# roncapat/UNIGE-TASI-path-planners

Measured on AMD Instinct MI355X. Metric: grid cells updated/sec (full plan + 100 replans), 4096^2 map, higher is better.
Workload: dtype f32

## Files before the change

unige-tasi-path-planners_amd/csrc/ufm_host.h:

```cpp
#pragma once

#define HIPCHK(expr)                                                      \
    do {                                                                  \
        hipError_t _e = (expr);                                           \
        if (_e != hipSuccess) return UFM_ERR_HIP_BASE - (int)_e;          \
    } while (0)

#include "ufm_route.h"
#include "ufm_path.h"

static_assert(RJOBS <= ROUTE_MAX_JOBS && RTMAX >= 3, "ufm_route.h places at most ROUTE_MAX_JOBS blocks");
constexpr RouteConfig ROUTE_CONFIG{T, RTMAX, RJOBS, ROUTE_MAX_RECTS, 65 * 65};

template <int V> using IntC = std::integral_constant<int, V>;
template <class F> void with_lower_op(int algo, F &&f) {
    if (algo == UFM_ALGO_FD) f(IntC<UFM_ALGO_FD>{});
    else if (algo == UFM_ALGO_SG) f(IntC<UFM_ALGO_SG>{});
    else f(IntC<ALGO_DFM1>{});
}
template <class F> void with_raise_op(int algo, bool follow_info, F &&f) {
    if (algo == UFM_ALGO_DFM && follow_info) f(IntC<ALGO_DFM1_INFO>{});
    else with_lower_op(algo, f);
}
template <class F> void with_elements(int algo, F &&f) {
// ... 962 lines not shown
            const int cnt = (p.h + 1) * (p.w + 1);
            if (pl.fused) put_rect(r.rb.rect[r.rb.nrect++], p);
            else k_clear_marks<<<(cnt + 255) / 256, 256, 0, stream>>>(P, p.m, p.x, p.y, p.w, p.h);
        }
        pending.resize(kept);
    }
    return UFM_OK;
}

int Engine::fused_end(float band) {
    ++pub_seq;
    k_replan_end<<<64, T * T, 0, stream>>>(P, iter[Q_RAISE], iter[Q_LOWER], band, h_ctr, h_flag, pub_seq);
    finalize_bp(1);
    HIPCHK(hipGetLastError());
    return wait_published();
}

int Engine::submit_block(StepRun &r) {
    const StepPlan &pl = r.plan;
    const bool batch = pl.route == Route::BlockBatch;
    RegionJobs rjs{};
    rjs.n = pl.njobs;
    const unsigned int seq = ++pub_seq;
    for (int i = 0; i < pl.njobs; ++i) {
        const RouteJob &pj = pl.job[i];
        RegionJob &j = rjs.j[i];
        if (batch) {
            j.rb.sb = step_begin_of(pj.map, 1, 0);
            j.rb.nrect = pj.nrect;
            std::memcpy(j.rb.rect, pj.rect, sizeof(pj.rect));
        } else {
            j.rb = r.rb;
        }
        j.rb.k_raise = iter[Q_RAISE]; j.rb.band = r.band;
        j.tx0 = pj.tx0; j.ntx = pj.ntx; j.ty0 = pj.ty0; j.nty = pj.nty;
        j.dyn = r.dyn_now; j.k_lower = iter[Q_LOWER]; j.max_sweeps = region_sweeps; j.debug = region_debug;
        j.slack = 255.0f * SQRT2F + 1.0f;
        j.delta = region_band > 0.0f ? region_band * 4.0f * mean_cost : INFINITY;
        j.map = pj.map; j.batch = batch ? 1 : 0; j.seq = seq;
    }
    if (pl.held_in_kernel) {
        const int first = r.rb.nrect - (int)lazy.size();
        for (size_t i = 0; i < lazy.size(); ++i) rjs.j[0].psrc[first + (int)i] = h_lazy + (size_t)lazy[i].slot * 4096;
        lazy.clear();
    }
    if (batch) {
        HIPCHK(hipMemsetAsync(&P.ctr->rbound, 0, offsetof(DevCounters, done_fail) + sizeof(int) - offsetof(DevCounters, rbound), stream));
        k_fill<<<1, 64, 0, stream>>>(reinterpret_cast<float *>(&P.ctr->qmin[Q_RAISE]), (size_t)1, INFINITY);
    }
    if (batch) flush_dyn(r);
    else { dyn_dev = r.dyn_now; r.dyn_pending = false; }
    const bool reg_timed = profiling && (region_runs & 7u) == 0u;
    if (reg_timed) for (auto &e : reg_ev) if (!e) HIPCHK(hipEventCreate(&e));
    with_raise_op(algo, dfm_follow_info, [&](auto a) {
        launch(k_replan_region<a()>, dim3(rjs.n), dim3(NTHR), stream, reg_timed ? reg_ev[0] : nullptr, reg_timed ? reg_ev[1] : nullptr, P, rjs, h_ctr, h_flag);
    });
    HIPCHK(hipGetLastError());
    last_active = 1;
    { int rc = wait_published(); if (rc != UFM_OK) return rc; }
    ufm_stats &st = r.st;
    st.region_launches = 1u;
    for (int i = 0; i < rjs.n; ++i) st.region_tiles += (uint32_t)(rjs.j[i].ntx * rjs.j[i].nty);
    if (reg_timed) {
        hipError_t q;
        while ((q = hipEventQuery(reg_ev[1])) == hipErrorNotReady) __builtin_ia32_pause();
        HIPCHK(q);
        HIPCHK(hipEventElapsedTime(&st.region_kernel_ms, reg_ev[0], reg_ev[1]));
        st.region_timed = 1u;
    }
    region_runs += (uint32_t)rjs.n;
    if (h_ctr->done) region_done += (uint32_t)rjs.n;
    else if (focused) {
        float qm;
        std::memcpy(&qm, &h_ctr->qmin[Q_RAISE], sizeof(float));
        r.skip_raise = !(qm < h_ctr->rbound);
    }
    return UFM_OK;
}

int Engine::continue_block(StepRun &r) {
    const int nr2 = r.skip_raise ? 1 : std::max(1, cont_raise), nl2 = cont_lower;
    last_active = 1;
    k_unpark<<<1, 1024, 0, stream>>>(P, Q_RAISE, iter[Q_RAISE], -1.0f);
    for (int i = 0; i < nr2; ++i) launch_relax(MODE_RAISE, -1.0f);
    k_raise_to_lower<<<1, 1024, 0, stream>>>(P, iter[Q_LOWER]);
    for (int i = 0; i < nl2; ++i) launch_relax(MODE_LOWER, INFINITY);
    { int rc = fused_end(r.band); if (rc != UFM_OK) return rc; }
    r.fast_done = h_ctr->done != 0;
    r.st.raise_launches += (uint32_t)nr2;
    r.st.launches += (uint32_t)(nr2 + nl2);
    r.skip_raise = false;
    ++region_cont; if (r.fast_done) ++region_cont_done;
    return UFM_OK;
}

int Engine::submit_graph(StepRun &r) {
    r.rb.k_raise = iter[Q_RAISE]; r.rb.band = r.band;
    hipGraphExec_t ge = nullptr;
    { int rc = replan_graph(r.nr, r.nl, r.band, &ge); if (rc != UFM_OK) return rc; }
    h_job->rb = r.rb; h_job->k_lower = iter[Q_LOWER]; h_job->seq = ++pub_seq;
    h_job->dyn = r.dyn_now; dyn_dev = r.dyn_now; r.dyn_pending = false;
    __atomic_thread_fence(__ATOMIC_RELEASE);
    HIPCHK(hipGraphLaunch(ge, stream));
    iter[Q_RAISE] += r.nr; iter[Q_LOWER] += r.nl;
    last_active = 1;
    return wait_published();
}

// ... 757 lines not shown
```

unige-tasi-path-planners_amd/csrc/ufm_region.h:

```cpp

constexpr int UFM_REGION_PRIO = 2;
#define UFM_REGION_SETPRIO(x) __builtin_amdgcn_s_setprio(x)
constexpr int UFM_REGION_IDLE_SLEEP = 8;
constexpr int UFM_REGION_IDLE_SLEEP_RAISE = 8;
constexpr int RTMAX = 128 / T;
constexpr int RN = RTMAX * T;
constexpr int RP = RN + 8;
constexpr int RCP = RN + 4;
constexpr int RBP = RN;
constexpr int TP = T / 4;
constexpr int RPW = RTMAX * TP / 4;
constexpr int RWW = (RPW * RPW + 31) / 32;
constexpr int RFRAME = 4 * RTMAX + 4;

struct RegionJob {
    ReplanBegin rb;
    DevDyn dyn;
    int tx0, ty0, ntx, nty;
    int k_lower;
    unsigned int seq;
    int max_sweeps;
    int debug;
    float slack;
    float delta;
    int map;
    int batch;
    const uint8_t *psrc[4];
};
constexpr int RJOBS = 8;
struct RegionJobs { int n; RegionJob j[RJOBS]; };

__device__ __forceinline__ int prio_read_fresh(const DevParams &P, int qz, int kk, int gt) {
    const unsigned long long v = __hip_atomic_load(&P.prio[(size_t)(qz * 2 + (kk & 1)) * P.NT + gt], __ATOMIC_RELAXED, __HIP_MEMORY_SCOPE_AGENT);
    return (int)(v >> 32) == 0x7FFFFFFF - kk ? (int)(unsigned int)v : INFBITS;
}

struct RegionShared {
    int wake[16][RWW];
    int ever[16][RWW];
    int renew[16][RWW];
    int tbp[RTMAX * RTMAX];
    int seed[16][RWW];
    int defer[2][16][RWW];
    int dprio[2][RTMAX * RTMAX];
    int tflag[RTMAX * RTMAX];
    int traised[RTMAX * RTMAX];
    int actL[RFRAME], actR[RFRAME];
    int soff[4];
    float sdist[4];
    float B0, rbound;
    float theta;
    float Bgate;
    int rmin;
    float Bsub;
    int swas[4];
    int idle, giveup, again, any_start_in;
    unsigned long long sweeps;
    int expanded;
    int m_r, m_l, done;
    int dkey;
    int dbg[8];
    int dbg2[8];
    unsigned long long tstamp[12];
};

__device__ __forceinline__ float region_start_key(const float *Gs, const RegionShared &S) {
    if (!S.any_start_in) return S.B0;
    float b = 0.0f;
#pragma unroll
    for (int i = 0; i < 4; ++i) {
        const int o = S.soff[i];
        if (o < 0) continue;
        const float g = Gs[o];
        if (g < INFINITY) b = fmaxf(b, g + S.sdist[i]);
    }
    return b > 0.0f ? b : INFINITY;
}

__device__ __forceinline__ float region_lower_bound(const float *Gs, const RegionShared &S) {
    if (!S.any_start_in) return S.B0;
    float b = 0.0f;
    bool pending = false;
#pragma unroll
    for (int i = 0; i < 4; ++i) {
        const int o = S.soff[i];
        if (o < 0) continue;
        const float g = Gs[o];
        if (g < INFINITY) b = fmaxf(b, g + S.sdist[i]);
        else if (S.swas[i]) pending = true;
    }
    if (pending) return fmaxf(b, S.rbound);
    return b > 0.0f ? b : INFINITY;
}

template <int ALGOF, int MODE>
__device__ void region_phase(const DevParams &P, const RegionJob &J, float *Gs, const uint8_t *Cb, uint8_t *Bb, RegionShared &S,
                             int thr, float hm, int focused, int goal_lx, int goal_ly) {
    constexpr int ALGO = algo_of(ALGOF);
    constexpr bool FOLLOW = (ALGOF & ALGO_FOLLOW_INFO) != 0;
    constexpr bool BPRAISE = MODE == MODE_RAISE && (!is_dfm<ALGO> || FOLLOW);
    const int tid = threadIdx.x, w = wave_index16(tid >> 6), lane = tid & 63;
    const int q = lane & 3, nd = lane >> 2;
    const int nprow = J.ntx * TP, npcol = J.nty * TP;
    unsigned long long wake_sel = 0ull;
    if (lane < 9) {
        const int dr = lane / 3 - 1, dc = lane % 3 - 1;
        wake_sel = ~0ull;
        if (dr < 0) wake_sel &= 0x000000000000FFFFull; else if (dr > 0) wake_sel &= 0xFFFF000000000000ull;
        if (dc < 0) wake_sel &= 0x000F000F000F000Full; else if (dc > 0) wake_sel &= 0xF000F000F000F000ull;
    }
    const int colour = ((nd >> 2) & 1) | ((nd & 1) << 1);
    const bool wt_lane = lane < 9;
    const int wt_dr = wt_lane ? lane / 3 - 1 : 0, wt_dc = wt_lane ? lane % 3 - 1 : 0;
    const int wt_ar = (w >> 2) + wt_dr, wt_ac = (w & 3) + wt_dc;
    const int wt_wave = ((wt_ar & 3) << 2) | (wt_ac & 3), wt_di = (wt_ar >> 2) * RPW + (wt_ac >> 2);
    const float sx = J.rb.sb.sx, sy = J.rb.sb.sy;
    const int rx0 = J.tx0 * T, ry0 = J.ty0 * T;
    int budget = J.max_sweeps;
    unsigned int my_sweeps = 0;
    auto cost_at = [=](int r, int c) { const int b = Cb[r * RCP + c]; return b >= thr ? INFINITY : (float)b; };
    const int so0 = __builtin_amdgcn_readfirstlane(S.soff[0]), so1 = __builtin_amdgcn_readfirstlane(S.soff[1]);
    const int so2 = __builtin_amdgcn_readfirstlane(S.soff[2]), so3 = __builtin_amdgcn_readfirstlane(S.soff[3]);
    const bool dbg_nogate = (J.debug & 1) != 0, dbg_count = (J.debug & 2) != 0;
    const float Bphase = (MODE == MODE_LOWER) ? S.Bgate : INFINITY;
    const float rb_phase = S.rbound + J.slack;
    const int nwords = min(RWW, (((nprow + 3) / 4 - 1) * RPW + (npcol + 3) / 4 + 31) / 32);
    UFM_REGION_SETPRIO(UFM_REGION_PRIO);
    for (;;) {
        bool took = false;
        bool vote = __hip_atomic_load(&S.giveup, __ATOMIC_RELAXED, __HIP_MEMORY_SCOPE_WORKGROUP) != 0;
        for (int wd = 0; wd < nwords && !vote; ++wd) {
            if (__hip_atomic_load(&S.wake[w][wd], __ATOMIC_RELAXED, __HIP_MEMORY_SCOPE_WORKGROUP) == 0) continue;
            int bits = 0;
            if (lane == 0) bits = atomicExch(&S.wake[w][wd], 0);
            bits = __builtin_amdgcn_readfirstlane(bits);
            if (!bits) continue;
            if (MODE == MODE_RAISE && lane == 0) S.ever[w][wd] |= bits;
            int seedbits = 0;
            if (BPRAISE) seedbits = __builtin_amdgcn_readfirstlane(S.seed[w][wd]) & bits;
            while (bits) {
                const int j = __ffs(bits) - 1;
                if (budget <= 0) {
                    if (lane == 0) {
                        __hip_atomic_fetch_or(&S.wake[w][wd], bits, __ATOMIC_RELAXED, __HIP_MEMORY_SCOPE_WORKGROUP);
                        __hip_atomic_store(&S.giveup, 1, __ATOMIC_RELAXED, __HIP_MEMORY_SCOPE_WORKGROUP);
                    }
                    vote = true;
                    break;
                }
                bits &= bits - 1;
                took = true;
                const int idx = wd * 32 + j;
                const int pr = (idx / RPW) * 4 + (w >> 2), pc = (idx % RPW) * 4 + (w & 3);
                if (pr >= nprow || pc >= npcol) continue;
                const int lx = pr * 4 + (nd >> 2), ly = pc * 4 + (nd & 3);
                const bool arith = BPRAISE && ((seedbits >> j) & 1);
                QuadConsts<ALGO> C;
                if (!BPRAISE || arith) C.load_at(cost_at, lx, ly, q, RP);
                float *ctr = Gs + (lx + 1) * RP + ly + 1;
                uint8_t *bpp = Bb + lx * RBP + ly;
                const int bpb = BPRAISE ? *bpp : BP_NONE;
                const int bqc = bpb >> 3, bsx = (bqc & 2) ? RP : -RP, bsy = (bqc & 1) ? 1 : -1;
                int bo1 = (bpb & 4) ? bsy : bsx, bo2 = bsx + bsy;
                if constexpr (is_dfm<ALGO>) dfm_bp_offsets<RP>(bpb, bo1, bo2);
                const bool bd1 = bpb & 1, bd2 = bpb & 2;
                const bool bnone = is_dfm<ALGO> && bpb == BP_NONE;
                const bool goal = (lx == goal_lx) & (ly == goal_ly);
                const int npr = pr + wt_dr, npc = pc + wt_dc, ni = idx + wt_di;
                const bool wt_ok = wt_lane & ((unsigned)npr < (unsigned)nprow) & ((unsigned)npc < (unsigned)npcol);
                const int nwave = wt_wave, nword = wt_ok ? (ni >> 5) : -1, nbit = 1 << (ni & 31);
                float hd = 0.0f;
                if (hm != 0.0f) {
                    const float x0 = (float)(rx0 + pr * 4), x1 = x0 + 3.0f, y0 = (float)(ry0 + pc * 4), y1 = y0 + 3.0f;
                    const float dx = fmaxf(fmaxf(x0 - sx, sx - x1), 0.0f), dy = fmaxf(fmaxf(y0 - sy, sy - y1), 0.0f);
                    hd = hm * hypotf(dx, dy) * 0.999f;
                }
                const int tl = (pr / TP) * J.nty + (pc / TP);
                const float B = Bphase;
                const int my_off = (lx + 1) * RP + ly + 1;
                const bool is_start = (my_off == so0) | (my_off == so1) | (my_off == so2) | (my_off == so3);
                const float rb = (MODE == MODE_RAISE && S.traised[tl]) ? INFINITY : rb_phase;
                asm volatile("" ::: "memory");
                float g = ctr[0];
                if (dbg_count && MODE == MODE_LOWER) {
                    const int sx_ = (q & 2) ? RP : -RP, sy_ = (q & 1) ? 1 : -1;
                    const bool fin = (g < INFINITY) | (ctr[sx_] < INFINITY) | (ctr[sy_] < INFINITY) | (ctr[sx_ + sy_] < INFINITY);
                    if (__builtin_amdgcn_ballot_w64(fin) == 0ull && lane == 0) atomicAdd(&S.dbg2[1], 1);
                }
                float dmin = INFINITY;
                float rmin_l = INFINITY;
                bool again = true, pch = false;
                [[maybe_unused]] bool held_last = false;
                [[maybe_unused]] float nv_last = INFINITY;
                [[maybe_unused]] const bool gate_free = is_start || B == INFINITY || dbg_nogate;
                unsigned long long chg = 0ull;
                int cnt = 0;
                for (int b = 0; b < 16 && again; ++b) {
                    asm volatile("" ::: "memory");
                    float nv;
                    if constexpr (BPRAISE) {
                        if (arith && b == 0) nv = quad_min(eval_quad_bp<ALGO, RP>(ctr, q, C, bpb));
                        else { const float p1 = ctr[bo1], p2 = ctr[bo2]; nv = ((bd1 && p1 == INFINITY) || (bd2 && p2 == INFINITY) || bnone) ? INFINITY : g; }
                    }
                    else nv = quad_min(eval_quad<ALGO, RP>(ctr, q, C));
                    if (goal) nv = 0.0f;
                    bool want, gate, doit;
                    if (MODE == MODE_LOWER) {
                        want = (nv != g);
                        gate = (nv + hd < B) || gate_free;
                        doit = want && gate && ((nv < g) || (colour == (cnt & 3)));
                        held_last = want && !gate; nv_last = nv;
                    } else {
                        if (is_dfm<ALGO>) want = (g < INFINITY) && (nv > g) && ((nv == INFINITY) || (__float_as_int(nv) - __float_as_int(g) > 8));
                        else want = (g < INFINITY) && (nv > g);
                        gate = !(g > rb) || dbg_nogate;
                        doit = want && gate;
                        if (want && !gate) dmin = fminf(dmin, g);
                        rmin_l = doit ? fminf(rmin_l, g) : rmin_l;
                        nv = INFINITY;
                    }
                    if (doit && q == 0) ctr[0] = nv;
                    const float gn = doit ? nv : g;
                    const unsigned long long mask = __builtin_amdgcn_ballot_w64(doit);
                    const unsigned long long wanted = __builtin_amdgcn_ballot_w64(want && gate);
                    g = gn;
                    pch |= mask != 0ull;
                    chg |= mask;
                    UFM_SWEEP_FENCE();
                    if ((mask & wake_sel) != 0ull && nword >= 0 && lane != 4)
                        __hip_atomic_fetch_or(&S.wake[nwave][nword], nbit, __ATOMIC_RELAXED, __HIP_MEMORY_SCOPE_WORKGROUP);
                    ++cnt;
                    again = wanted != 0ull;
                }
                budget -= cnt; my_sweeps += cnt;
                if (pch && lane == 0) S.tflag[tl] = 1;
                if (MODE == MODE_LOWER && held_last) dmin = nv_last;
                if ((chg & wake_sel) != 0ull && nword >= 0) __hip_atomic_fetch_or(&S.renew[nwave][nword], nbit, __ATOMIC_RELAXED, __HIP_MEMORY_SCOPE_WORKGROUP);
                if (BPRAISE && arith) {
                    const unsigned long long held = __builtin_amdgcn_ballot_w64(dmin < INFINITY);
                    if (lane == 0 && held == 0ull) S.seed[w][wd] &= ~(1 << j);
                }
                if (MODE == MODE_RAISE && rmin_l < INFINITY && q == 0) { atomicMin(&S.rmin, __float_as_int(rmin_l)); S.traised[tl] = 1; }
                if (dbg_count && lane == 0) { atomicAdd(&S.dbg[MODE == MODE_LOWER ? 5 : 4], 1); atomicAdd(&S.dbg[MODE == MODE_LOWER ? 7 : 6], cnt); if (!pch) atomicAdd(&S.dbg2[MODE == MODE_LOWER ? 0 : 2], 1); }
                if (again && lane == 0) __hip_atomic_fetch_or(&S.wake[w][wd], 1 << j, __ATOMIC_RELAXED, __HIP_MEMORY_SCOPE_WORKGROUP);
                if (dmin < INFINITY && q == 0) {
                    atomicAdd(&S.dbg[MODE == MODE_LOWER ? 0 : 1], 1);
                    atomicMin(&S.dprio[MODE == MODE_LOWER ? 0 : 1][tl], __float_as_int(dmin));
                    if (MODE == MODE_LOWER) atomicMin(&S.dkey, __float_as_int(dmin + hd));
                    __hip_atomic_fetch_or(&S.defer[MODE == MODE_LOWER ? 0 : 1][w][wd], 1 << j, __ATOMIC_RELAXED, __HIP_MEMORY_SCOPE_WORKGROUP);
                }
            }
        }
        if (took && !vote) continue;
        if (!vote) {
            if (lane == 0) atomicAdd(&S.idle, 1);
            UFM_REGION_SETPRIO(0);
            for (;;) {
                __builtin_amdgcn_s_sleep(BPRAISE ? UFM_REGION_IDLE_SLEEP_RAISE : UFM_REGION_IDLE_SLEEP);
                const int idle_now = __hip_atomic_load(&S.idle, __ATOMIC_RELAXED, __HIP_MEMORY_SCOPE_WORKGROUP);
                const int gave_up_now = __hip_atomic_load(&S.giveup, __ATOMIC_RELAXED, __HIP_MEMORY_SCOPE_WORKGROUP);
                int any = 0;
#pragma unroll
                for (int wd = 0; wd < RWW; ++wd) any |= __hip_atomic_load(&S.wake[w][wd], __ATOMIC_RELAXED, __HIP_MEMORY_SCOPE_WORKGROUP);
                if (idle_now >= 16 || gave_up_now != 0) { vote = true; break; }
                if (any) { if (lane == 0) atomicSub(&S.idle, 1); break; }
            }
            UFM_REGION_SETPRIO(UFM_REGION_PRIO);
            if (!vote) continue;
        }
        __syncthreads();
        int mine = 0;
#pragma unroll
        for (int wd = 0; wd < RWW; ++wd) mine |= __hip_atomic_load(&S.wake[w][wd], __ATOMIC_RELAXED, __HIP_MEMORY_SCOPE_WORKGROUP);
        const int work = __syncthreads_or(mine != 0);
        const int gave_up = __hip_atomic_load(&S.giveup, __ATOMIC_RELAXED, __HIP_MEMORY_SCOPE_WORKGROUP);
        if (gave_up || !work) break;
        if (tid == 0) S.idle = 0;
        __syncthreads();
    }
    UFM_REGION_SETPRIO(0);
    if (lane == 0 && my_sweeps) atomicAdd(&S.sweeps, (unsigned long long)my_sweeps);
    __syncthreads();
    if (tid == 0) S.idle = 0;
    __syncthreads();
}

template <int ALGOF>
__global__ __launch_bounds__(NTHR) void k_replan_region(DevParams P, RegionJobs JS, DevCounters *host, unsigned int *flag) {
    constexpr int ALGO = algo_of(ALGOF);
    __shared__ float Gs[(RN + 2) * RP];
    __shared__ uint8_t Cb[(RN + 1) * RCP];
    __shared__ __attribute__((aligned(16))) uint8_t Bb[RN * RBP];
    __shared__ RegionShared S;
    __shared__ int s_last;
#ifdef UFM_REGION_NG0
    constexpr int NG0 = UFM_REGION_NG0;
#else
    constexpr int NG0 = (46 * 1024) / (TT * 4);
#endif
    __shared__ float G0c[NG0 * TT];
    __shared__ int s_wbl[RTMAX * RTMAX];
    __shared__ int s_nwb;
    __shared__ uint8_t s_pmask[4096];
    __shared__ int s_simd[16];
    __shared__ unsigned long long s_tb[8];
    constexpr bool CELLS = is_dfm<ALGO>;
    constexpr int COFF = CELLS ? 0 : 1;
    const int tid = threadIdx.x;
    const RegionJob &J = JS.j[blockIdx.x];
    const int m = J.map, gt0 = m * P.NTm;
    const int ntl = J.ntx * J.nty;
    const int nty_magic = (65536 + J.nty - 1) / J.nty;
    const int rx0 = J.tx0 * T, ry0 = J.ty0 * T, rnx = J.ntx * T, rny = J.nty * T;

    const unsigned long long t_begin = wall_clock64();
#define STAMP(k) do { if (tid == 0 && (J.debug & 2)) s_tb[k] = wall_clock64(); } while (0)
    STAMP(0);
    if ((tid & 63) == 0 && (J.debug & 2)) s_simd[tid >> 6] = (int)__builtin_amdgcn_s_getreg((1 << 11) | (4 << 6) | 4);
    const float hm = J.dyn.hm;
    const int thr = J.dyn.thr, focused = J.dyn.focused;
    int r_first = -1;
    for (int r = J.rb.nrect - 1; r >= 0; --r) if (J.psrc[r]) r_first = r;
    const bool one_fused = J.rb.nrect == 1 && r_first == 0 && !J.batch;
    int pb0[4] = {0, 0, 0, 0};
    if (r_first >= 0) {
        const int n0 = J.rb.rect[r_first][3] * J.rb.rect[r_first][4];
#pragma unroll
        for (int c = 0; c < 4; ++c) { const int e = tid + c * NTHR; if (e < n0) pb0[c] = J.psrc[r_first][e]; }
    }
    float sg = INFINITY;
    int se_x = -1, se_y = -1;
    {
        const int e = tid == 0 ? J.rb.sb.start[0] : (tid == 1 ? J.rb.sb.start[1] : (tid == 2 ? J.rb.sb.start[2] : (tid == 3 ? J.rb.sb.start[3] : -1)));
        if (e >= 0) { se_x = e / P.EY; se_y = e - se_x * P.EY; sg = P.G[gaddr(P, m, se_x, se_y)]; }
    }
    const int n_pending = P.ctr->scount;
    const int goal_x = P.goal[2 * m], goal_y = P.goal[2 * m + 1];
    STAMP(1);
    const int wv = __builtin_amdgcn_readfirstlane(tid >> 6), ln = tid & 63;
    {
        const int crow = rnx + COFF, ccol = rny + COFF;
        constexpr int KP = (RN + 64) / 64, KR = (RN + 16) / 16;
        const uint8_t *cbase = P.cost + (size_t)m * P.cstride;
        uint8_t cv[KP * KR];
#pragma unroll
        for (int j = 0; j < KP; ++j) {
            const int c = j * 64 + ln, cy = ry0 + c - COFF;
            const bool cok = c < ccol && cy >= 0 && cy < P.W;
#pragma unroll
            for (int k = 0; k < KR; ++k) {
                const int r = wv + 16 * k, cx = rx0 + r - COFF;
                cv[j * KR + k] = 255;
                if (j * 64 < ccol && r < crow && cx >= 0 && cx < P.L && cok) cv[j * KR + k] = cbase[(size_t)cx * P.W + cy];
            }
        }
        constexpr int CPT = TT / 256, KT = RTMAX * RTMAX * CPT / 16;
        float4 gv[KT];
        unsigned int bv[KT];
#pragma unroll
        for (int k = 0; k < KT; ++k) {
            const int pc = wv + 16 * k, tl = pc / CPT;
            if (tl >= ntl) continue;
            const int ti = (tl * nty_magic) >> 16, tj = tl - ti * J.nty, v = (pc - tl * CPT) * 64 + ln;
            const size_t gt = (size_t)(gt0 + (J.tx0 + ti) * P.TY + J.ty0 + tj);
            gv[k] = reinterpret_cast<const float4 *>(P.G + gt * TT)[v];
            bv[k] = reinterpret_cast<const unsigned int *>(P.bp + gt * TT)[v];
        }
        static_assert(4 * RN + 4 <= NTHR, "one frame element per thread");
        float fv = INFINITY;
        int fo = -1;
        if (tid < 2 * (rny + 2) + 2 * rnx) {
            int hx, hy;
// ... 29 lines not shown
    for (int r = 0; r < J.rb.nrect; ++r) {
        if (!J.psrc[r]) continue;
        const int *qr = J.rb.rect[r];
        const int px = qr[1], py = qr[2], pw = qr[3], ph = qr[4];
        const unsigned pw_magic = ((1u << 20) + (unsigned)pw - 1u) / (unsigned)pw;
        __syncthreads();
        STAMP(2);
#pragma unroll
        for (int c = 0; c < 4; ++c) {
            const int e = tid + c * NTHR;
            if (e >= pw * ph) continue;
            const int i = (int)(((unsigned)e * pw_magic) >> 20), j = e - i * pw;
            uint8_t *cb = &Cb[(px + i - rx0 + COFF) * RCP + (py + j - ry0 + COFF)];
            const uint8_t nv = (r == r_first) ? (uint8_t)pb0[c] : J.psrc[r][e];
            const uint8_t ch = *cb != nv;
            s_pmask[e] = ch;
            if (ch) { *cb = nv; P.cost[(size_t)m * P.cstride + (size_t)(px + i) * P.W + (py + j)] = nv; cost_window_store(P, m, px + i, py + j, nv); }
        }
        __syncthreads();
        STAMP(3);
        const int ne = CELLS ? pw * ph : (pw + 1) * (ph + 1);
        if (one_fused) {
            const int ew = CELLS ? pw : pw + 1;
            const unsigned ew_magic = ((1u << 20) + (unsigned)ew - 1u) / (unsigned)ew;
            int cnt = 0;
            for (int e = tid; e < ne; e += NTHR) {
                const int i = (int)(((unsigned)e * ew_magic) >> 20), j = e - i * ew;
                bool ch;
                if (!CELLS) ch = (i > 0 && j > 0 && s_pmask[(i - 1) * pw + j - 1]) || (i > 0 && j < pw && s_pmask[(i - 1) * pw + j]) ||
                                 (i < ph && j > 0 && s_pmask[i * pw + j - 1]) || (i < ph && j < pw && s_pmask[i * pw + j]);
                else ch = s_pmask[i * pw + j];
                cnt += ch ? 1 : 0;
            }
            for (int o = 32; o; o >>= 1) cnt += __shfl_xor(cnt, o);
            if ((tid & 63) == 0 && cnt) atomicAdd(&P.num_updated[m], (unsigned int)cnt);
        } else {
            for (int base = 0; base < ne; base += NTHR) patch_seed<!CELLS>(P, m, s_pmask, px, py, pw, ph, base + tid);
        }
    }
    if (J.rb.nrect && J.psrc[J.rb.nrect - 1]) __syncthreads();
    STAMP(4);
    if (tid == 0 && !J.batch) *P.dyn = J.dyn;
    if (!J.batch) step_begin(P, J.rb.sb);
    if (!one_fused)
        for (int r = 0; r < J.rb.nrect; ++r) {
            const int *qr = J.rb.rect[r];
            for (int e = tid; e < (qr[3] + 1) * (qr[4] + 1); e += NTHR) clear_mark(P, qr[0], qr[1], qr[2], qr[3], qr[4], e);
        }
    for (int i = tid; i < (int)(sizeof(RegionShared) / sizeof(int)); i += NTHR) reinterpret_cast<int *>(&S)[i] = 0;
    __syncthreads();
    STAMP(5);
    for (int i = tid; i < 2 * RTMAX * RTMAX; i += NTHR) (&S.dprio[0][0])[i] = INFBITS;
    for (int i = tid; i < RFRAME; i += NTHR) { S.actL[i] = INFBITS; S.actR[i] = INFBITS; }
    if (tid == 0) { S.rmin = INFBITS; S.m_r = INFBITS; }
    {
        const int n = one_fused ? n_pending : P.ctr->scount;
        for (int i = tid; i < n; i += NTHR) {
            const int gt = P.slist[i];
            if (gt / P.NTm != m) continue;
            const int tx = (gt - gt0) / P.TY, ty = (gt - gt0) - tx * P.TY;
            P.sflag[gt] = 0;
            if (tx < J.tx0 || tx >= J.tx0 + J.ntx || ty < J.ty0 || ty >= J.ty0 + J.nty) activate(P, Q_RAISE, J.rb.k_raise, gt, 0);
        }
        __syncthreads();
        STAMP(6);
        if (tid == 0 && !J.batch) { P.ctr->scount = 0; P.ctr->done = 0; }
        if (tid < 64) {
            float key = 0.0f, dist = 0.0f;
            int off = -1;
            if (se_x >= 0) {
                dist = hm * hypotf(J.rb.sb.sx - (float)se_x, J.rb.sb.sy - (float)se_y);
                if (sg < INFINITY) key = sg + dist;
                if (se_x >= rx0 && se_x < rx0 + rnx && se_y >= ry0 && se_y < ry0 + rny) off = (se_x - rx0 + 1) * RP + (se_y - ry0 + 1);
            }
            if (tid < 4) { S.soff[tid] = off; S.sdist[tid] = dist; }
            const bool in = __builtin_amdgcn_ballot_w64(off >= 0) != 0ull;
            float b0 = fmaxf(key, __shfl_xor(key, 1));
            b0 = fmaxf(b0, __shfl_xor(b0, 2));
            if (tid == 0) {
                b0 = b0 > 0.0f ? b0 : INFINITY;
                S.B0 = b0;
                S.rbound = focused ? b0 + J.rb.band : INFINITY;
                S.any_start_in = in ? 1 : 0;
            }
        }
    }

    if (tid == 0) { S.tstamp[0] = t_begin; S.tstamp[1] = wall_clock64(); S.tstamp[2] = S.tstamp[1]; }
    __syncthreads();
    for (int r = 0; r < J.rb.nrect; ++r) {
        const int *qr = J.rb.rect[r];
        const int ex0 = qr[1] - rx0, ex1 = qr[1] + qr[4] - (CELLS ? 1 : 0) - rx0, ey0 = qr[2] - ry0, ey1 = qr[2] + qr[3] - (CELLS ? 1 : 0) - ry0;
        const int p0 = max(ex0, 0) / 4, p1 = min(ex1, rnx - 1) / 4, c0 = max(ey0, 0) / 4, c1 = min(ey1, rny - 1) / 4;
        const int np = (p1 - p0 + 1) * (c1 - c0 + 1);
        for (int i = tid; i < np; i += NTHR) {
            const int pr = p0 + i / (c1 - c0 + 1), pc = c0 + i % (c1 - c0 + 1);
            const int ni = (pr >> 2) * RPW + (pc >> 2);
            atomicOr(&S.wake[((pr & 3) << 2) | (pc & 3)][ni >> 5], 1 << (ni & 31));
            atomicOr(&S.seed[((pr & 3) << 2) | (pc & 3)][ni >> 5], 1 << (ni & 31));
            S.traised[(pr / TP) * J.nty + pc / TP] = 1;
        }
    }
    if (tid < 4) S.swas[tid] = (S.soff[tid] >= 0 && Gs[S.soff[tid]] < INFINITY) ? 1 : 0;
    __syncthreads();
    const int goal_lx = goal_x - rx0, goal_ly = goal_y - ry0;

    for (int round = 0;; ++round) {
        for (;;) {
            region_phase<ALGOF, MODE_RAISE>(P, J, Gs, Cb, Bb, S, thr, hm, focused, goal_lx, goal_ly);
            const int again_t = __syncthreads_or(tid < ntl && S.traised[tid] && S.dprio[1][tid] != INFBITS) && !S.giveup;
            __syncthreads();
            if (!again_t) break;
            for (int i = tid; i < 16 * RWW; i += NTHR) { (&S.wake[0][0])[i] |= (&S.defer[1][0][0])[i]; (&S.defer[1][0][0])[i] = 0; }
            for (int i = tid; i < RTMAX * RTMAX; i += NTHR) S.dprio[1][i] = INFBITS;
            __syncthreads();
        }
        if (tid == 0 && round == 0) S.tstamp[3] = wall_clock64();
        for (int i = tid; i < 16 * RWW; i += NTHR) {
            (&S.wake[0][0])[i] |= (&S.ever[0][0])[i] | (&S.defer[0][0][0])[i];
            (&S.ever[0][0])[i] = 0; (&S.defer[0][0][0])[i] = 0;
        }
        for (int i = tid; i < RTMAX * RTMAX; i += NTHR) S.dprio[0][i] = INFBITS;
        if (tid == 0) {
            S.dkey = INFBITS;
            S.Bsub = focused ? region_lower_bound(Gs, S) : INFINITY;
            S.theta = (round == 0) ? ((S.rmin != INFBITS) ? __int_as_float(S.rmin) + J.delta : INFINITY) : S.theta;
            S.Bgate = fminf(S.Bsub + J.slack, S.theta);
        }
        __syncthreads();
        for (int sub = 0;; ++sub) {
            region_phase<ALGO, MODE_LOWER>(P, J, Gs, Cb, Bb, S, thr, hm, focused, goal_lx, goal_ly);
            if (tid == 0) {
                const float B = focused ? region_lower_bound(Gs, S) : INFINITY;
                const int m = S.dkey;
                bool again = !S.giveup && m != INFBITS && (__int_as_float(m) < B || B == INFINITY);
                if (again && sub >= 4096) { again = false; S.giveup = 1; }
                S.again = again ? 1 : 0;
                S.Bsub = B;
                if (again) S.theta = fmaxf(S.theta, __int_as_float(m)) + J.delta;
                S.Bgate = fminf(S.Bsub + J.slack, S.theta);
            }
            __syncthreads();
            const int again_l = S.again;
            __syncthreads();
            if (!again_l) break;
            if (tid == 0) ++S.dbg[2];
            for (int i = tid; i < 16 * RWW; i += NTHR) { (&S.wake[0][0])[i] |= (&S.defer[0][0][0])[i]; (&S.defer[0][0][0])[i] = 0; }
            for (int i = tid; i < RTMAX * RTMAX; i += NTHR) S.dprio[0][i] = INFBITS;
            if (tid == 0) S.dkey = INFBITS;
            __syncthreads();
        }
        if (tid < ntl && S.dprio[1][tid] != INFBITS) atomicMin(&S.m_r, S.dprio[1][tid]);
        __syncthreads();
        if (tid == 0) {
            const float B = focused ? region_lower_bound(Gs, S) : INFINITY;
            const int m = S.m_r;
            S.m_r = INFBITS;
            bool again = !S.giveup && focused && m != INFBITS && __int_as_float(m) < B + J.slack;
            if (again && round >= 14) { again = false; S.giveup = 1; }
            if (again) S.rbound = fmaxf(B, S.rbound) + J.rb.band;
            S.again = again ? 1 : 0;
        }
        __syncthreads();
        const int again_r = S.again;
        __syncthreads();
        if (!again_r) break;
        if (tid == 0) ++S.dbg[3];
        for (int i = tid; i < 16 * RWW; i += NTHR) { (&S.wake[0][0])[i] |= (&S.defer[1][0][0])[i]; (&S.defer[1][0][0])[i] = 0; }
        for (int i = tid; i < RTMAX * RTMAX; i += NTHR) S.dprio[1][i] = INFBITS;
        __syncthreads();
    }

    if (tid == 0) S.tstamp[4] = wall_clock64();
    auto frame_index = [&](int ti, int tj) {
        if (ti < 0) return tj + 1;
        if (ti >= J.ntx) return (J.nty + 2) + tj + 1;
        if (tj < 0) return 2 * (J.nty + 2) + ti;
        return 2 * (J.nty + 2) + J.ntx + ti;
    };
    static_assert(NTHR == 1024 && TT % 64 == 0 && RBP % 4 == 0, "the block kernel deals its staging and write-back out by wave");
    constexpr int UPT = TT / 64;
    const int wvw = __builtin_amdgcn_readfirstlane(tid >> 6), lnw = tid & 63;
    if (tid < 64) {
        const bool has = tid < ntl && S.tflag[tid];
        const unsigned long long hm_ = __builtin_amdgcn_ballot_w64(has);
        if (has) s_wbl[__popcll(hm_ & ((1ull << tid) - 1ull))] = tid;
        if (tid == 0) s_nwb = __popcll(hm_);
    }
    __syncthreads();
    const int nunits = s_nwb * UPT;
    auto unit_tile = [&](int u, int &k, int &part, int &tl, int &ti, int &tj) {
        k = u / UPT; part = u - k * UPT; tl = __builtin_amdgcn_readfirstlane(s_wbl[k]);
        ti = (tl * nty_magic) >> 16; tj = tl - ti * J.nty;
    };
    {
        typedef __attribute__((address_space(3))) void *lds_ptr;
        typedef const __attribute__((address_space(1))) void *glb_ptr;
#pragma unroll 1
        for (int u = wvw; u < nunits; u += 16) {
            int k, part, tl, ti, tj;
            unit_tile(u, k, part, tl, ti, tj);
            if (k >= NG0) continue;
            const size_t gt = (size_t)(gt0 + (J.tx0 + ti) * P.TY + J.ty0 + tj);
            __builtin_amdgcn_global_load_lds((glb_ptr)(P.G + gt * TT + part * 64 + lnw), (lds_ptr)(G0c + k * TT + part * 64), 4, 0, 0);
        }
        asm volatile("s_waitcnt vmcnt(0)" ::: "memory");
    }
    __syncthreads();
    int n_exp = 0;
#pragma unroll 1
    for (int u = wvw; u < nunits; u += 16) {
        int k, part, tl, ti, tj;
        unit_tile(u, k, part, tl, ti, tj);
        const int e = part * 64 + lnw;
        const int tx = J.tx0 + ti, ty = J.ty0 + tj, gt = gt0 + tx * P.TY + ty;
        const int io_r = e / T, io_c = e % T;
        float gl0;
        if (k < NG0) gl0 = G0c[k * TT + e];
        else { gl0 = P.G[(size_t)gt * TT + e]; P.Gprev[(size_t)gt * TT + e] = gl0; }
        const float gf = Gs[(ti * T + io_r + 1) * RP + tj * T + io_c + 1];
        if (gf == gl0) continue;
        ++n_exp;
        P.G[(size_t)gt * TT + e] = gf;
        const int er = (io_r == 0) ? -1 : ((io_r == T - 1) ? 1 : 0);
        const int ec = (io_c == 0) ? -1 : ((io_c == T - 1) ? 1 : 0);
        const bool rok = er && tx + er >= 0 && tx + er < P.TX, cok = ec && ty + ec >= 0 && ty + ec < P.TY;
// ... 12 lines not shown
            if (lowered) return lo < fmaxf(fmaxf(a, b), c);
            const float fa = a < INFINITY ? a : -INFINITY, fb = b < INFINITY ? b : -INFINITY, fc = c < INFINITY ? c : -INFINITY;
            return gl0 < fmaxf(fmaxf(fa, fb), fc);
        };
        if (out_r) {
            const float *h = Gs + (lxr + er) * RP + lyc;
            if (concerned(h[cl], h[0], h[ch])) atomicMin(lowered ? &S.actL[frame_index(ti + er, tj)] : &S.actR[frame_index(ti + er, tj)], pb);
        }
        if (out_c) {
            const float *h = Gs + lxr * RP + lyc + ec;
            if (concerned(h[rl * RP], h[0], h[rh * RP])) atomicMin(lowered ? &S.actL[frame_index(ti, tj + ec)] : &S.actR[frame_index(ti, tj + ec)], pb);
        }
        if (rok && cok && (out_r || out_c)) {
            const int di = ti + er, dj = tj + ec;
            if (di < 0 || di >= J.ntx || dj < 0 || dj >= J.nty) {
                const float hv = Gs[(lxr + er) * RP + lyc + ec];
                if (concerned(hv, hv, hv)) atomicMin(lowered ? &S.actL[frame_index(di, dj)] : &S.actR[frame_index(di, dj)], pb);
            }
        }
    }
    if (n_exp) atomicAdd(&S.expanded, n_exp);
    __syncthreads();
    for (int i = tid; i < 2 * (J.nty + 2) + 2 * J.ntx; i += NTHR) {
        int ti, tj;
        if (i < J.nty + 2) { ti = -1; tj = i - 1; }
        else if (i < 2 * (J.nty + 2)) { ti = J.ntx; tj = i - (J.nty + 2) - 1; }
        else if (i < 2 * (J.nty + 2) + J.ntx) { ti = i - 2 * (J.nty + 2); tj = -1; }
        else { ti = i - 2 * (J.nty + 2) - J.ntx; tj = J.nty; }
        const int tx = J.tx0 + ti, ty = J.ty0 + tj;
        if (tx < 0 || ty < 0 || tx >= P.TX || ty >= P.TY) continue;
        const int gt = gt0 + tx * P.TY + ty;
        if (S.actR[i] != INFBITS) activate(P, Q_RAISE, J.rb.k_raise, gt, S.actR[i]);
        if (S.actL[i] != INFBITS) activate(P, Q_LOWER, J.k_lower, gt, S.actL[i]);
    }
    for (int tl = tid; tl < ntl; tl += NTHR) {
        const int gt = gt0 + (J.tx0 + tl / J.nty) * P.TY + J.ty0 + tl % J.nty;
        if (S.dprio[0][tl] != INFBITS) park_tile(P, Q_LOWER, gt, S.dprio[0][tl]);
        if (S.dprio[1][tl] != INFBITS) park_tile(P, Q_RAISE, gt, S.dprio[1][tl]);
    }
    if (S.giveup) {
        for (int i = tid; i < 16 * RWW * 32; i += NTHR) {
            const int w = i / (RWW * 32), r = i % (RWW * 32);
            if (!(S.wake[w][r >> 5] & (1 << (r & 31)))) continue;
            const int pr = (r / RPW) * 4 + (w >> 2), pc = (r % RPW) * 4 + (w & 3);
            if (pr >= J.ntx * TP || pc >= J.nty * TP) continue;
            const int gt = gt0 + (J.tx0 + pr / TP) * P.TY + J.ty0 + pc / TP;
            activate(P, Q_RAISE, J.rb.k_raise, gt, 0);
            activate(P, Q_LOWER, J.k_lower, gt, 0);
        }
    }
    if (J.batch) __threadfence(); else __builtin_amdgcn_fence(__ATOMIC_RELEASE, "workgroup");
    __syncthreads();

    if (tid == 0) S.tstamp[5] = wall_clock64();
    if (tid == 0) { S.m_r = INFBITS; S.m_l = INFBITS; }
    __syncthreads();
    {
        const float B = focused ? region_start_key(Gs, S) : INFINITY;
        int mr = INFBITS, ml = INFBITS;
        const int nr = __hip_atomic_load(&P.ctr->cnt[Q_RAISE][J.rb.k_raise % 3], __ATOMIC_RELAXED, __HIP_MEMORY_SCOPE_AGENT);
        const int npr = __hip_atomic_load(&P.ctr->npark[Q_RAISE], __ATOMIC_RELAXED, __HIP_MEMORY_SCOPE_AGENT);
        const int nl = __hip_atomic_load(&P.ctr->cnt[Q_LOWER][J.k_lower % 3], __ATOMIC_RELAXED, __HIP_MEMORY_SCOPE_AGENT);
        const int npl = __hip_atomic_load(&P.ctr->npark[Q_LOWER], __ATOMIC_RELAXED, __HIP_MEMORY_SCOPE_AGENT);
        auto mine = [&](int gt) { return (unsigned)gt < (unsigned)P.NT && gt / P.NTm == m; };
        for (int i = tid; i < nr; i += NTHR) {
            const int gt = __hip_atomic_load(&P.cand[(size_t)(Q_RAISE * 3 + J.rb.k_raise % 3) * P.NT + i], __ATOMIC_RELAXED, __HIP_MEMORY_SCOPE_AGENT);
            if (mine(gt)) mr = min(mr, prio_read_fresh(P, Q_RAISE, J.rb.k_raise, gt));
        }
        for (int i = tid; i < npr; i += NTHR) {
            const int gt = __hip_atomic_load(&P.park[(size_t)(Q_RAISE * 2) * P.NT + i], __ATOMIC_RELAXED, __HIP_MEMORY_SCOPE_AGENT);
            if (mine(gt)) mr = min(mr, __hip_atomic_load(&P.pprio[Q_RAISE * P.NT + gt], __ATOMIC_RELAXED, __HIP_MEMORY_SCOPE_AGENT));
        }
        auto lower_key = [&](int gt, int pbits) {
            if (pbits == INFBITS) return INFINITY;
            return __int_as_float(pbits) + (focused ? tile_heuristic(P, m, (gt - gt0) / P.TY, (gt - gt0) % P.TY) : 0.0f);
        };
        float kl = INFINITY;
        for (int i = tid; i < nl; i += NTHR) {
            const int gt = __hip_atomic_load(&P.cand[(size_t)(Q_LOWER * 3 + J.k_lower % 3) * P.NT + i], __ATOMIC_RELAXED, __HIP_MEMORY_SCOPE_AGENT);
            if (mine(gt)) kl = fminf(kl, lower_key(gt, prio_read_fresh(P, Q_LOWER, J.k_lower, gt)));
        }
        for (int i = tid; i < npl; i += NTHR) {
            const int gt = __hip_atomic_load(&P.park[(size_t)(Q_LOWER * 2) * P.NT + i], __ATOMIC_RELAXED, __HIP_MEMORY_SCOPE_AGENT);
            if (mine(gt)) kl = fminf(kl, lower_key(gt, __hip_atomic_load(&P.pprio[Q_LOWER * P.NT + gt], __ATOMIC_RELAXED, __HIP_MEMORY_SCOPE_AGENT)));
        }
        ml = kl < INFINITY ? __float_as_int(kl) : INFBITS;
        if (mr != INFBITS) atomicMin(&S.m_r, mr);
        if (ml != INFBITS) atomicMin(&S.m_l, ml);
        __syncthreads();
        if (tid == 0) {
            bool done;
            if (focused && B < INFINITY) done = !(__int_as_float(S.m_r) < B) && !(__int_as_float(S.m_l) < B);
            else done = (S.m_r == INFBITS && S.m_l == INFBITS) && (J.batch || (nr == 0 && nl == 0));
            if (S.giveup) done = false;
            S.done = done ? 1 : 0;
            unsigned int upd = 0;
            if (P.consume[m]) { upd = P.num_updated[m]; P.num_updated[m] = 0; }
            if (!J.batch) {
                P.ctr->done = S.done;
                P.ctr->rbound = S.rbound;
                P.ctr->qmin[Q_RAISE] = S.m_r;
                P.ctr->updated = upd;
                P.ctr->tile_visits += (unsigned long long)ntl;
                P.ctr->raise_visits += (unsigned long long)ntl / 2;
                P.ctr->tile_iters += S.sweeps / 16;
                P.ctr->elem_evals += 16ull * S.sweeps;
                if (done) P.ctr->expanded = (unsigned long long)S.expanded;
            } else {
                if (!done) atomicAdd(&P.ctr->done_fail, 1);
                if (S.m_r != INFBITS && __int_as_float(S.m_r) < S.rbound) atomicMin(&P.ctr->qmin[Q_RAISE], 0);
                atomicMax(reinterpret_cast<int *>(&P.ctr->rbound), __float_as_int(S.rbound));
                atomicAdd(&P.ctr->updated, upd);
                atomicAdd(&P.ctr->tile_visits, (unsigned long long)ntl);
                atomicAdd(&P.ctr->raise_visits, (unsigned long long)ntl / 2);
                atomicAdd(&P.ctr->tile_iters, S.sweeps / 16);
                atomicAdd(&P.ctr->elem_evals, 16ull * S.sweeps);
                if (done) atomicAdd(&P.ctr->expanded, (unsigned long long)S.expanded);
            }
            if (J.debug & 2) {
                int nd0 = 0, nd1 = 0, m0 = INFBITS, m1 = INFBITS;
                for (int i = 0; i < ntl; ++i) { if (S.dprio[0][i] != INFBITS) { ++nd0; m0 = min(m0, S.dprio[0][i]); } if (S.dprio[1][i] != INFBITS) { ++nd1; m1 = min(m1, S.dprio[1][i]); } }
                int *d = P.lmax;
                d[0] = __float_as_int(B); d[1] = __float_as_int(S.B0); d[2] = __float_as_int(S.rbound); d[3] = S.m_r; d[4] = S.m_l;
                d[5] = nr; d[6] = nl; d[7] = npr; d[8] = npl; d[9] = S.done; d[10] = S.giveup; d[11] = (int)S.sweeps; d[12] = S.expanded;
                d[13] = nd0; d[14] = m0; d[15] = nd1; d[16] = m1; d[17] = S.any_start_in;
                for (int i = 0; i < 4; ++i) d[18 + i] = S.soff[i] >= 0 ? __float_as_int(Gs[S.soff[i]]) : -1;
                for (int i = 0; i < 8; ++i) d[22 + i] = S.dbg[i];
                S.tstamp[6] = wall_clock64();
                for (int i = 1; i < 7; ++i) d[30 + i] = (int)(S.tstamp[i] - S.tstamp[0]);
                d[37] = 0; d[38] = 0;
                for (int i = 1; i < 8; ++i) d[40 + i] = (int)(s_tb[i] - s_tb[0]);
                for (int i = 0; i < 16; ++i) d[50 + i] = s_simd[i];
                for (int i = 0; i < 8; ++i) d[70 + i] = S.dbg2[i];
            }
        }
        __syncthreads();
    }
    if (!S.done) {
#pragma unroll 1
        for (int u = wvw; u < nunits; u += 16) {
            int k, part, tl, ti, tj;
            unit_tile(u, k, part, tl, ti, tj);
            const int e = part * 64 + lnw;
            const int gt = gt0 + (J.tx0 + ti) * P.TY + J.ty0 + tj;
            if (k < NG0) P.Gprev[(size_t)gt * TT + e] = G0c[k * TT + e];
            if (e == 0) {
                P.fresh[gt] = 0;
                if (atomicAdd(&P.touched[gt], 1) == 0) P.tlist[atomicAdd(&P.ctr->tcount, 1)] = gt;
            }
        }
    }
    if (J.batch) __threadfence();
    __syncthreads();
    if (J.batch) {
        if (tid == 0) s_last = (atomicAdd(&P.ctr->fin_blocks, 1) == (int)gridDim.x - 1);
        __syncthreads();
        if (s_last) {
            __threadfence();
            if (tid == 0) {
                P.ctr->fin_blocks = 0;
                P.ctr->scount = 0;
                P.ctr->done = __hip_atomic_load(&P.ctr->done_fail, __ATOMIC_RELAXED, __HIP_MEMORY_SCOPE_AGENT) == 0 ? 1 : 0;
            }
            __threadfence();
            __syncthreads();
        }
    }
    if (!J.batch || s_last) {
        const int *src = reinterpret_cast<const int *>(P.ctr);
        int *dst = reinterpret_cast<int *>(host);
        for (int i = tid; i < (int)(sizeof(DevCounters) / sizeof(int)); i += NTHR)
            dst[i] = __hip_atomic_load(&src[i], __ATOMIC_RELAXED, __HIP_MEMORY_SCOPE_AGENT);
        __syncthreads();
        if (tid == 0) {
            if (J.debug & 2) P.lmax[37] = (int)(wall_clock64() - S.tstamp[0]);
            __hip_atomic_store(flag, J.seq, __ATOMIC_RELEASE, __HIP_MEMORY_SCOPE_SYSTEM);
        }
    }

    {
        const int w = wave_index16(tid >> 6), lane = tid & 63, q = lane & 3, nd = lane >> 2;
        const int nprow = J.ntx * TP, npcol = J.nty * TP;
        auto cost_at = [=](int r, int c) { const int b = Cb[r * RCP + c]; return b >= thr ? INFINITY : (float)b; };
        for (int wd = 0; wd < RWW; ++wd) {
            int bits = __builtin_amdgcn_readfirstlane(S.renew[w][wd]);
            while (bits) {
                const int j = __ffs(bits) - 1;
                bits &= bits - 1;
                const int idx = wd * 32 + j;
                const int pr = (idx / RPW) * 4 + (w >> 2), pc = (idx % RPW) * 4 + (w & 3);
                if (pr >= nprow || pc >= npcol) continue;
                const int lx = pr * 4 + (nd >> 2), ly = pc * 4 + (nd & 3);
                QuadConsts<ALGO> C;
                C.load_at(cost_at, lx, ly, q, RP);
                const LaneEval le = eval_quad_w<ALGO, RP>(Gs + (lx + 1) * RP + ly + 1, q, C);
                const float nv = quad_min(le.r);
                const int bq = quad_min_int(bp_byte<ALGO>(le, q, C, le.r == nv)), b = bp_of_key<ALGO>(bq);
                if (q == 0) Bb[lx * RBP + ly] = (uint8_t)((lx == goal_lx && ly == goal_ly) ? BP_NONE : b);
                if (lane == 0) S.tbp[(pr / TP) * J.nty + pc / TP] = 1;
            }
        }
        __syncthreads();
    }
    if (tid < 64) {
        const bool has = tid < ntl && S.tbp[tid];
        const unsigned long long hm_ = __builtin_amdgcn_ballot_w64(has);
        if (has) s_wbl[__popcll(hm_ & ((1ull << tid) - 1ull))] = tid;
        if (tid == 0) s_nwb = __popcll(hm_);
    }
    __syncthreads();
    const int nunits_bp = s_nwb * UPT;
#pragma unroll 1
    for (int u = wvw; u < nunits_bp; u += 16) {
        int k, part, tl, ti, tj;
        unit_tile(u, k, part, tl, ti, tj);
        const int e = part * 64 + lnw;
        P.bp[(size_t)(gt0 + (J.tx0 + ti) * P.TY + J.ty0 + tj) * TT + e] = Bb[(ti * T + e / T) * RBP + tj * T + e % T];
    }
    if (J.debug & 2) {
        __syncthreads();
        if (tid == 0) P.lmax[38] = (int)(wall_clock64() - S.tstamp[0]);
    }
}
```

Measured before the change: 585.8 million.

## Specialize region kernel on heuristic/debug flags and shard dkey reduction per word

Adds a FORM template parameter to the region replan kernel so that the heuristic and debug code paths are compiled out when unused, removing runtime branches, wall-clock reads and debug atomics. Replaces the single shared-memory atomicMin on dkey with a per-wave/per-word pkey array. That array is reduced into dkey after each lower phase, which is meant to cut contention on one LDS word. This adds extra LDS footprint, an extra reduction pass and a barrier per sub-iteration, and the host now picks among three kernel instantiations.

```diff
diff --git a/unige-tasi-path-planners_amd/csrc/ufm_host.h b/unige-tasi-path-planners_amd/csrc/ufm_host.h
--- a/unige-tasi-path-planners_amd/csrc/ufm_host.h
+++ b/unige-tasi-path-planners_amd/csrc/ufm_host.h
@@ -1038,8 +1038,14 @@
     else { dyn_dev = r.dyn_now; r.dyn_pending = false; }
     const bool reg_timed = profiling && (region_runs & 7u) == 0u;
     if (reg_timed) for (auto &e : reg_ev) if (!e) HIPCHK(hipEventCreate(&e));
+    const int form = region_debug ? (RF_HEUR | RF_DEBUG) : (r.dyn_now.hm != 0.0f ? RF_HEUR : 0);
     with_raise_op(algo, dfm_follow_info, [&](auto a) {
-        launch(k_replan_region<a()>, dim3(rjs.n), dim3(NTHR), stream, reg_timed ? reg_ev[0] : nullptr, reg_timed ? reg_ev[1] : nullptr, P, rjs, h_ctr, h_flag);
+        auto go = [&](auto f) {
+            launch(k_replan_region<a(), f()>, dim3(rjs.n), dim3(NTHR), stream, reg_timed ? reg_ev[0] : nullptr, reg_timed ? reg_ev[1] : nullptr, P, rjs, h_ctr, h_flag);
+        };
+        if (form == 0) go(IntC<0>{});
+        else if (form == RF_HEUR) go(IntC<RF_HEUR>{});
+        else go(IntC<(RF_HEUR | RF_DEBUG)>{});
     });
     HIPCHK(hipGetLastError());
     last_active = 1;
diff --git a/unige-tasi-path-planners_amd/csrc/ufm_region.h b/unige-tasi-path-planners_amd/csrc/ufm_region.h
--- a/unige-tasi-path-planners_amd/csrc/ufm_region.h
+++ b/unige-tasi-path-planners_amd/csrc/ufm_region.h
@@ -29,6 +29,7 @@
 };
 constexpr int RJOBS = 8;
 struct RegionJobs { int n; RegionJob j[RJOBS]; };
+constexpr int RF_HEUR = 1, RF_DEBUG = 2;
 
 __device__ __forceinline__ int prio_read_fresh(const DevParams &P, int qz, int kk, int gt) {
     const unsigned long long v = __hip_atomic_load(&P.prio[(size_t)(qz * 2 + (kk & 1)) * P.NT + gt], __ATOMIC_RELAXED, __HIP_MEMORY_SCOPE_AGENT);
@@ -59,6 +60,7 @@
     int expanded;
     int m_r, m_l, done;
     int dkey;
+    int pkey[16][RWW * 32];
     int dbg[8];
     int dbg2[8];
     unsigned long long tstamp[12];
@@ -93,10 +95,11 @@
     return b > 0.0f ? b : INFINITY;
 }
 
-template <int ALGOF, int MODE>
+template <int ALGOF, int MODE, int FORM>
 __device__ void region_phase(const DevParams &P, const RegionJob &J, float *Gs, const uint8_t *Cb, uint8_t *Bb, RegionShared &S,
                              int thr, float hm, int focused, int goal_lx, int goal_ly) {
     constexpr int ALGO = algo_of(ALGOF);
+    constexpr bool HEUR = (FORM & RF_HEUR) != 0, DBG = (FORM & RF_DEBUG) != 0;
     constexpr bool FOLLOW = (ALGOF & ALGO_FOLLOW_INFO) != 0;
     constexpr bool BPRAISE = MODE == MODE_RAISE && (!is_dfm<ALGO> || FOLLOW);
     const int tid = threadIdx.x, w = wave_index16(tid >> 6), lane = tid & 63;
@@ -121,7 +124,7 @@
     auto cost_at = [=](int r, int c) { const int b = Cb[r * RCP + c]; return b >= thr ? INFINITY : (float)b; };
     const int so0 = __builtin_amdgcn_readfirstlane(S.soff[0]), so1 = __builtin_amdgcn_readfirstlane(S.soff[1]);
     const int so2 = __builtin_amdgcn_readfirstlane(S.soff[2]), so3 = __builtin_amdgcn_readfirstlane(S.soff[3]);
-    const bool dbg_nogate = (J.debug & 1) != 0, dbg_count = (J.debug & 2) != 0;
+    const bool dbg_nogate = DBG && (J.debug & 1) != 0, dbg_count = DBG && (J.debug & 2) != 0;
     const float Bphase = (MODE == MODE_LOWER) ? S.Bgate : INFINITY;
     const float rb_phase = S.rbound + J.slack;
     const int nwords = min(RWW, (((nprow + 3) / 4 - 1) * RPW + (npcol + 3) / 4 + 31) / 32);
@@ -170,7 +173,7 @@
                 const bool wt_ok = wt_lane & ((unsigned)npr < (unsigned)nprow) & ((unsigned)npc < (unsigned)npcol);
                 const int nwave = wt_wave, nword = wt_ok ? (ni >> 5) : -1, nbit = 1 << (ni & 31);
                 float hd = 0.0f;
-                if (hm != 0.0f) {
+                if (HEUR && hm != 0.0f) {
                     const float x0 = (float)(rx0 + pr * 4), x1 = x0 + 3.0f, y0 = (float)(ry0 + pc * 4), y1 = y0 + 3.0f;
                     const float dx = fmaxf(fmaxf(x0 - sx, sx - x1), 0.0f), dy = fmaxf(fmaxf(y0 - sy, sy - y1), 0.0f);
                     hd = hm * hypotf(dx, dy) * 0.999f;
@@ -243,10 +246,11 @@
                 if (MODE == MODE_RAISE && rmin_l < INFINITY && q == 0) { atomicMin(&S.rmin, __float_as_int(rmin_l)); S.traised[tl] = 1; }
                 if (dbg_count && lane == 0) { atomicAdd(&S.dbg[MODE == MODE_LOWER ? 5 : 4], 1); atomicAdd(&S.dbg[MODE == MODE_LOWER ? 7 : 6], cnt); if (!pch) atomicAdd(&S.dbg2[MODE == MODE_LOWER ? 0 : 2], 1); }
                 if (again && lane == 0) __hip_atomic_fetch_or(&S.wake[w][wd], 1 << j, __ATOMIC_RELAXED, __HIP_MEMORY_SCOPE_WORKGROUP);
+                if (MODE == MODE_LOWER && lane == 0) __hip_atomic_store(&S.pkey[w][idx], INFBITS, __ATOMIC_RELAXED, __HIP_MEMORY_SCOPE_WORKGROUP);
                 if (dmin < INFINITY && q == 0) {
-                    atomicAdd(&S.dbg[MODE == MODE_LOWER ? 0 : 1], 1);
+                    if (DBG) atomicAdd(&S.dbg[MODE == MODE_LOWER ? 0 : 1], 1);
                     atomicMin(&S.dprio[MODE == MODE_LOWER ? 0 : 1][tl], __float_as_int(dmin));
-                    if (MODE == MODE_LOWER) atomicMin(&S.dkey, __float_as_int(dmin + hd));
+                    if (MODE == MODE_LOWER) atomicMin(&S.pkey[w][idx], __float_as_int(dmin + hd));
                     __hip_atomic_fetch_or(&S.defer[MODE == MODE_LOWER ? 0 : 1][w][wd], 1 << j, __ATOMIC_RELAXED, __HIP_MEMORY_SCOPE_WORKGROUP);
                 }
             }
@@ -285,9 +289,10 @@
     __syncthreads();
 }
 
-template <int ALGOF>
+template <int ALGOF, int FORM>
 __global__ __launch_bounds__(NTHR) void k_replan_region(DevParams P, RegionJobs JS, DevCounters *host, unsigned int *flag) {
     constexpr int ALGO = algo_of(ALGOF);
+    constexpr bool HEUR = (FORM & RF_HEUR) != 0, DBG = (FORM & RF_DEBUG) != 0;
     __shared__ float Gs[(RN + 2) * RP];
     __shared__ uint8_t Cb[(RN + 1) * RCP];
     __shared__ __attribute__((aligned(16))) uint8_t Bb[RN * RBP];
@@ -313,11 +318,12 @@
     const int nty_magic = (65536 + J.nty - 1) / J.nty;
     const int rx0 = J.tx0 * T, ry0 = J.ty0 * T, rnx = J.ntx * T, rny = J.nty * T;
 
-    const unsigned long long t_begin = wall_clock64();
-#define STAMP(k) do { if (tid == 0 && (J.debug & 2)) s_tb[k] = wall_clock64(); } while (0)
+    const int debug = DBG ? J.debug : 0;
+    const unsigned long long t_begin = DBG ? wall_clock64() : 0ull;
+#define STAMP(k) do { if (DBG && tid == 0 && (debug & 2)) s_tb[k] = wall_clock64(); } while (0)
     STAMP(0);
-    if ((tid & 63) == 0 && (J.debug & 2)) s_simd[tid >> 6] = (int)__builtin_amdgcn_s_getreg((1 << 11) | (4 << 6) | 4);
-    const float hm = J.dyn.hm;
+    if (DBG && (tid & 63) == 0 && (debug & 2)) s_simd[tid >> 6] = (int)__builtin_amdgcn_s_getreg((1 << 11) | (4 << 6) | 4);
+    const float hm = HEUR ? J.dyn.hm : 0.0f;
     const int thr = J.dyn.thr, focused = J.dyn.focused;
     int r_first = -1;
     for (int r = J.rb.nrect - 1; r >= 0; --r) if (J.psrc[r]) r_first = r;
@@ -453,6 +459,7 @@
     STAMP(5);
     for (int i = tid; i < 2 * RTMAX * RTMAX; i += NTHR) (&S.dprio[0][0])[i] = INFBITS;
     for (int i = tid; i < RFRAME; i += NTHR) { S.actL[i] = INFBITS; S.actR[i] = INFBITS; }
+    for (int i = tid; i < 16 * RWW * 32; i += NTHR) (&S.pkey[0][0])[i] = INFBITS;
     if (tid == 0) { S.rmin = INFBITS; S.m_r = INFBITS; }
     {
         const int n = one_fused ? n_pending : P.ctr->scount;
@@ -470,7 +477,7 @@
             float key = 0.0f, dist = 0.0f;
             int off = -1;
             if (se_x >= 0) {
-                dist = hm * hypotf(J.rb.sb.sx - (float)se_x, J.rb.sb.sy - (float)se_y);
+                if (HEUR) dist = hm * hypotf(J.rb.sb.sx - (float)se_x, J.rb.sb.sy - (float)se_y);
                 if (sg < INFINITY) key = sg + dist;
                 if (se_x >= rx0 && se_x < rx0 + rnx && se_y >= ry0 && se_y < ry0 + rny) off = (se_x - rx0 + 1) * RP + (se_y - ry0 + 1);
             }
@@ -487,7 +494,7 @@
         }
     }
 
-    if (tid == 0) { S.tstamp[0] = t_begin; S.tstamp[1] = wall_clock64(); S.tstamp[2] = S.tstamp[1]; }
+    if (DBG && tid == 0) { S.tstamp[0] = t_begin; S.tstamp[1] = wall_clock64(); S.tstamp[2] = S.tstamp[1]; }
     __syncthreads();
     for (int r = 0; r < J.rb.nrect; ++r) {
         const int *qr = J.rb.rect[r];
@@ -508,7 +515,7 @@
 
     for (int round = 0;; ++round) {
         for (;;) {
-            region_phase<ALGOF, MODE_RAISE>(P, J, Gs, Cb, Bb, S, thr, hm, focused, goal_lx, goal_ly);
+            region_phase<ALGOF, MODE_RAISE, FORM>(P, J, Gs, Cb, Bb, S, thr, hm, focused, goal_lx, goal_ly);
             const int again_t = __syncthreads_or(tid < ntl && S.traised[tid] && S.dprio[1][tid] != INFBITS) && !S.giveup;
             __syncthreads();
             if (!again_t) break;
@@ -516,7 +523,7 @@
             for (int i = tid; i < RTMAX * RTMAX; i += NTHR) S.dprio[1][i] = INFBITS;
             __syncthreads();
         }
-        if (tid == 0 && round == 0) S.tstamp[3] = wall_clock64();
+        if (DBG && tid == 0 && round == 0) S.tstamp[3] = wall_clock64();
         for (int i = tid; i < 16 * RWW; i += NTHR) {
             (&S.wake[0][0])[i] |= (&S.ever[0][0])[i] | (&S.defer[0][0][0])[i];
             (&S.ever[0][0])[i] = 0; (&S.defer[0][0][0])[i] = 0;
@@ -530,7 +537,9 @@
         }
         __syncthreads();
         for (int sub = 0;; ++sub) {
-            region_phase<ALGO, MODE_LOWER>(P, J, Gs, Cb, Bb, S, thr, hm, focused, goal_lx, goal_ly);
+            region_phase<ALGO, MODE_LOWER, FORM>(P, J, Gs, Cb, Bb, S, thr, hm, focused, goal_lx, goal_ly);
+            for (int i = tid; i < 16 * RWW * 32; i += NTHR) { const int k = (&S.pkey[0][0])[i]; if (k != INFBITS) atomicMin(&S.dkey, k); }
+            __syncthreads();
             if (tid == 0) {
                 const float B = focused ? region_lower_bound(Gs, S) : INFINITY;
                 const int m = S.dkey;
@@ -545,7 +554,7 @@
             const int again_l = S.again;
             __syncthreads();
             if (!again_l) break;
-            if (tid == 0) ++S.dbg[2];
+            if (DBG && tid == 0) ++S.dbg[2];
             for (int i = tid; i < 16 * RWW; i += NTHR) { (&S.wake[0][0])[i] |= (&S.defer[0][0][0])[i]; (&S.defer[0][0][0])[i] = 0; }
             for (int i = tid; i < RTMAX * RTMAX; i += NTHR) S.dprio[0][i] = INFBITS;
             if (tid == 0) S.dkey = INFBITS;
@@ -566,13 +575,13 @@
         const int again_r = S.again;
         __syncthreads();
         if (!again_r) break;
-        if (tid == 0) ++S.dbg[3];
+        if (DBG && tid == 0) ++S.dbg[3];
         for (int i = tid; i < 16 * RWW; i += NTHR) { (&S.wake[0][0])[i] |= (&S.defer[1][0][0])[i]; (&S.defer[1][0][0])[i] = 0; }
         for (int i = tid; i < RTMAX * RTMAX; i += NTHR) S.dprio[1][i] = INFBITS;
         __syncthreads();
     }
 
-    if (tid == 0) S.tstamp[4] = wall_clock64();
+    if (DBG && tid == 0) S.tstamp[4] = wall_clock64();
     auto frame_index = [&](int ti, int tj) {
         if (ti < 0) return tj + 1;
         if (ti >= J.ntx) return (J.nty + 2) + tj + 1;
@@ -691,7 +700,7 @@
     if (J.batch) __threadfence(); else __builtin_amdgcn_fence(__ATOMIC_RELEASE, "workgroup");
     __syncthreads();
 
-    if (tid == 0) S.tstamp[5] = wall_clock64();
+    if (DBG && tid == 0) S.tstamp[5] = wall_clock64();
     if (tid == 0) { S.m_r = INFBITS; S.m_l = INFBITS; }
     __syncthreads();
     {
@@ -756,7 +765,7 @@
                 atomicAdd(&P.ctr->elem_evals, 16ull * S.sweeps);
                 if (done) atomicAdd(&P.ctr->expanded, (unsigned long long)S.expanded);
             }
-            if (J.debug & 2) {
+            if (DBG && (debug & 2)) {
                 int nd0 = 0, nd1 = 0, m0 = INFBITS, m1 = INFBITS;
                 for (int i = 0; i < ntl; ++i) { if (S.dprio[0][i] != INFBITS) { ++nd0; m0 = min(m0, S.dprio[0][i]); } if (S.dprio[1][i] != INFBITS) { ++nd1; m1 = min(m1, S.dprio[1][i]); } }
                 int *d = P.lmax;
@@ -812,7 +821,7 @@
             dst[i] = __hip_atomic_load(&src[i], __ATOMIC_RELAXED, __HIP_MEMORY_SCOPE_AGENT);
         __syncthreads();
         if (tid == 0) {
-            if (J.debug & 2) P.lmax[37] = (int)(wall_clock64() - S.tstamp[0]);
+            if (DBG && (debug & 2)) P.lmax[37] = (int)(wall_clock64() - S.tstamp[0]);
             __hip_atomic_store(flag, J.seq, __ATOMIC_RELEASE, __HIP_MEMORY_SCOPE_SYSTEM);
         }
     }
@@ -856,7 +865,7 @@
         const int e = part * 64 + lnw;
         P.bp[(size_t)(gt0 + (J.tx0 + ti) * P.TY + J.ty0 + tj) * TT + e] = Bb[(ti * T + e / T) * RBP + tj * T + e % T];
     }
-    if (J.debug & 2) {
+    if (DBG && (debug & 2)) {
         __syncthreads();
         if (tid == 0) P.lmax[38] = (int)(wall_clock64() - S.tstamp[0]);
     }
```

Result: faster. 602.2 million (median of 6 runs) (+2.8%).
